# Arcadia-Science/arcadia-microscopy-tools

Hardware: AMD Instinct MI355X
Metric: fields-of-view/sec (4x2048^2 uint16) end-to-end segment+props (higher is better)
Workload: dtype f64; 1 GPU; configs[2]: synthetic 4-channel 2048x2048 uint16 FOVs, DAPI Gaussian+Otsu+open/close+EDT+peak markers+watershed nuclei (SEEDED relief, seeds_first: marker pixels spread first in raster order, cannot tie; SURVEY A.8's plain -EDT relief with exact ties is reported under sublines.a8_exact) + clear_border/relabel + morphology and 4-channel intensity regionprops; mode=weak scaling, 192 FOVs per GPU per step, streams_per_gpu=4, fovs_per_launch=48, max_cells_per_fov=2048, distinct_fovs_per_gpu=8, resident_in_hbm=True

## Files before the change

arcadia_microscopy_tools_amd/csrc/amt_common.h:

```cpp
#pragma once
#include <hip/hip_runtime.h>

#include <cstdarg>
#include <cstdint>
#include <cstdio>
#include <cstring>

#include "../../include/amt_hip.h"
#include "amt_scratch_plan.h"

struct amt_ctx {
    int device;
    hipStream_t stream;
    bool own_stream;
    char* arena;
    size_t arena_cap;
    char* mailbox;
    size_t mailbox_cap;
    size_t mailbox_off;
    int num_cus;
    hipStream_t aux[3];
    hipStream_t aux_own[3];
    hipEvent_t ev[4];
    bool aux_ready;
    int fork;
    size_t plan_off[AMT_SCRATCH_SLOTS];
    size_t plan_len[AMT_SCRATCH_SLOTS];
    int plan_count;
    size_t plan_total;
    bool plan_valid;
    unsigned long long* dbg_first;
};

int amt_fork(amt_ctx* ctx);
int amt_join(amt_ctx* ctx);

void amt_set_error(const char* fmt, ...);

#define AMT_HIP_CHECK(expr)                                                                      \
    do {                                                                                         \
        hipError_t _e = (expr);                                                                  \
        if (_e != hipSuccess) {                                                                  \
            amt_set_error("%s failed: %s (%s:%d)", #expr, hipGetErrorString(_e), __FILE__, __LINE__); \
            return AMT_EHIP;                                                                     \
        }                                                                                        \
    } while (0)

// ... 41 lines not shown
    for (long long v : f) {
        if (n > (SIZE_MAX >> 1) / (size_t)v) return SIZE_MAX >> 1;
        n *= (size_t)v;
    }
    return n;
}
static inline size_t amt_esize(int dtype) {
    switch (dtype) {
        case AMT_U8: return 1;
        case AMT_U16: return 2;
        case AMT_I32: case AMT_F32: return 4;
        case AMT_F64: case AMT_I64: return 8;
        default: return 0;
    }
}
int amt_check_operands(const char* op, const amt_operand* ops, int n);
#define AMT_CHECK_OPERANDS(op, ...)                                                              \
    do {                                                                                         \
        const amt_operand _ops[] = {__VA_ARGS__};                                                \
        AMT_TRY(amt_check_operands(op, _ops, (int)(sizeof(_ops) / sizeof(_ops[0]))));            \
    } while (0)

struct amt_scratch : amt_scratch_plan {
    amt_ctx* ctx;
    explicit amt_scratch(amt_ctx* c) : ctx(c) {}
    int commit();
};
int amt_param_upload(amt_ctx* ctx, void* dev_dst, const void* host_src, size_t bytes);

__host__ __device__ static inline size_t amt_align(size_t n, size_t a = 256) { return (n + a - 1) / a * a; }

static inline int amt_set_device(amt_ctx* ctx) {
    if (!ctx) {
        amt_set_error("null context");
        return AMT_EINVAL;
// ... 49 lines not shown
```

arcadia_microscopy_tools_amd/csrc/amt_ctx.hip:

```cpp
#include "amt_common.h"

#include <cstdlib>

static thread_local char g_err[1024] = "";

void amt_set_error(const char* fmt, ...) {
    va_list ap;
    va_start(ap, fmt);
    vsnprintf(g_err, sizeof(g_err), fmt, ap);
    va_end(ap);
}

int amt_check_operands(const char* op, const amt_operand* ops, int n) {
    for (int i = 0; i < n; ++i) {
        const amt_operand& a = ops[i];
        if (!a.ptr || !a.bytes) continue;
        const uintptr_t a0 = reinterpret_cast<uintptr_t>(a.ptr);
        const uintptr_t a1 = a.bytes > UINTPTR_MAX - a0 ? UINTPTR_MAX : a0 + a.bytes;
        for (int j = i + 1; j < n; ++j) {
            const amt_operand& b = ops[j];
            if (!b.ptr || !b.bytes || !(a.output || b.output)) continue;
            const uintptr_t b0 = reinterpret_cast<uintptr_t>(b.ptr);
            const uintptr_t b1 = b.bytes > UINTPTR_MAX - b0 ? UINTPTR_MAX : b0 + b.bytes;
            if (a1 <= b0 || b1 <= a0) continue;
            const amt_operand& o = a.output ? a : b;
            const amt_operand& x = a.output ? b : a;
            const bool allowed = (a.output && !b.output && ((a.inplace >> j) & 1u)) ||
                                 (b.output && !a.output && ((b.inplace >> i) & 1u));
// ... 67 lines not shown
    return AMT_OK;
}

extern "C" int amt_ctx_create(int device, amt_ctx** out) { return ctx_create_common(device, nullptr, true, out); }

extern "C" int amt_ctx_create_on_stream(int device, void* hip_stream, amt_ctx** out) {
    return ctx_create_common(device, (hipStream_t)hip_stream, false, out);
}

extern "C" int amt_ctx_destroy(amt_ctx* ctx) {
    if (!ctx) return AMT_OK;
    (void)hipSetDevice(ctx->device);
    (void)hipStreamSynchronize(ctx->stream);
    if (ctx->arena) (void)hipFree(ctx->arena);
    if (ctx->dbg_first) (void)hipFree(ctx->dbg_first);
    if (ctx->mailbox) (void)hipHostFree(ctx->mailbox);
    if (ctx->aux_ready) {
        for (int i = 0; i < 3; ++i) (void)hipStreamDestroy(ctx->aux_own[i]);
        for (int i = 0; i < 4; ++i) (void)hipEventDestroy(ctx->ev[i]);
    }
    if (ctx->own_stream) (void)hipStreamDestroy(ctx->stream);
    delete ctx;
    return AMT_OK;
}

extern "C" int amt_device_name(amt_ctx* ctx, char* buf, int buflen) {
    AMT_TRY(amt_set_device(ctx));
    AMT_REQUIRE(buf && buflen > 0, "amt_device_name: bad buffer");
    hipDeviceProp_t prop;
    AMT_HIP_CHECK(hipGetDeviceProperties(&prop, ctx->device));
    snprintf(buf, (size_t)buflen, "%s (%s, %d CUs)", prop.name, prop.gcnArchName, prop.multiProcessorCount);
    return AMT_OK;
}

static bool poison_enabled() {
    static int v = -1;
    if (v < 0) {
        const char* e = getenv("AMT_DEBUG_POISON");
        v = (e && e[0] == '1') ? 1 : 0;
    }
    return v == 1;
}

int amt_scratch::commit() {
    AMT_REQUIRE(!overflow, "scratch plan: more than %d buffers declared", AMT_SCRATCH_SLOTS);
    ctx->plan_valid = false;
    const size_t total_bytes = total + 4096;
    if (total_bytes > ctx->arena_cap) {
        AMT_HIP_CHECK(hipStreamSynchronize(ctx->stream));
        if (ctx->arena) AMT_HIP_CHECK(hipFree(ctx->arena));
        ctx->arena = nullptr;
        ctx->arena_cap = 0;
        size_t cap = total_bytes + total_bytes / 4;
        hipError_t e = hipMalloc((void**)&ctx->arena, cap);
        if (e != hipSuccess) {
            amt_set_error("scratch arena allocation of %zu bytes failed: %s", cap, hipGetErrorString(e));
// ... 116 lines not shown
        AMT_HIP_CHECK(hipStreamSynchronize(ctx->stream));
        return AMT_OK;
    }
    if (ctx->mailbox_off + need > ctx->mailbox_cap) {
        AMT_HIP_CHECK(hipStreamSynchronize(ctx->stream));
        ctx->mailbox_off = 0;
    }
    char* slot = ctx->mailbox + ctx->mailbox_off;
    ctx->mailbox_off += need;
    memcpy(slot, host_src, bytes);
    AMT_HIP_CHECK(hipMemcpyAsync(dev_dst, slot, bytes, hipMemcpyHostToDevice, ctx->stream));
    return AMT_OK;
}

extern "C" int amt_malloc(amt_ctx* ctx, size_t bytes, void** dptr) {
    AMT_TRY(amt_set_device(ctx));
    AMT_REQUIRE(dptr != nullptr, "amt_malloc: dptr is null");
    if (bytes == 0) bytes = 256;
    hipError_t e = hipMalloc(dptr, bytes);
    if (e != hipSuccess) {
        amt_set_error("hipMalloc(%zu) failed: %s", bytes, hipGetErrorString(e));
        return AMT_ENOMEM;
    }
    if (poison_enabled()) {
        AMT_HIP_CHECK(hipMemsetAsync(*dptr, 0xCD, bytes, ctx->stream));
        AMT_HIP_CHECK(hipStreamSynchronize(ctx->stream));
    }
    return AMT_OK;
}

extern "C" int amt_free(amt_ctx* ctx, void* dptr) {
    AMT_TRY(amt_set_device(ctx));
    if (dptr) AMT_HIP_CHECK(hipFree(dptr));
    return AMT_OK;
}

extern "C" int amt_memcpy_h2d(amt_ctx* ctx, void* dst, const void* src, size_t bytes) {
    AMT_TRY(amt_set_device(ctx));
    if (bytes) AMT_HIP_CHECK(hipMemcpyAsync(dst, src, bytes, hipMemcpyHostToDevice, ctx->stream));
    return AMT_OK;
}
extern "C" int amt_memcpy_d2h(amt_ctx* ctx, void* dst, const void* src, size_t bytes) {
    AMT_TRY(amt_set_device(ctx));
    if (bytes) AMT_HIP_CHECK(hipMemcpyAsync(dst, src, bytes, hipMemcpyDeviceToHost, ctx->stream));
    return AMT_OK;
}
extern "C" int amt_memcpy_d2d(amt_ctx* ctx, void* dst, const void* src, size_t bytes) {
    AMT_TRY(amt_set_device(ctx));
    if (bytes) AMT_HIP_CHECK(hipMemcpyAsync(dst, src, bytes, hipMemcpyDeviceToDevice, ctx->stream));
    return AMT_OK;
}
extern "C" int amt_memset(amt_ctx* ctx, void* dst, int value, size_t bytes) {
    AMT_TRY(amt_set_device(ctx));
    if (bytes) AMT_HIP_CHECK(hipMemsetAsync(dst, value, bytes, ctx->stream));
    return AMT_OK;
}
extern "C" int amt_sync(amt_ctx* ctx) {
    AMT_TRY(amt_set_device(ctx));
    AMT_HIP_CHECK(hipStreamSynchronize(ctx->stream));
    return AMT_OK;
}

extern "C" int amt_ctx_stream(amt_ctx* ctx, void** hip_stream) {
    AMT_REQUIRE(ctx && hip_stream, "amt_ctx_stream: null argument");
    *hip_stream = (void*)ctx->stream;
    return AMT_OK;
}

extern "C" int amt_stream_wait(amt_ctx* ctx, amt_ctx* other) {
    AMT_TRY(amt_set_device(ctx));
    AMT_REQUIRE(other != nullptr, "amt_stream_wait: other is null");
    AMT_REQUIRE(other->device == ctx->device, "amt_stream_wait: contexts on different devices");
    hipEvent_t ev;
    AMT_HIP_CHECK(hipEventCreateWithFlags(&ev, hipEventDisableTiming));
    AMT_HIP_CHECK(hipEventRecord(ev, other->stream));
    AMT_HIP_CHECK(hipStreamWaitEvent(ctx->stream, ev, 0));
    AMT_HIP_CHECK(hipEventDestroy(ev));
    return AMT_OK;
}

extern "C" int amt_event_create(amt_ctx* ctx, void** event) {
    AMT_TRY(amt_set_device(ctx));
    AMT_REQUIRE(event != nullptr, "amt_event_create: event is null");
    hipEvent_t ev;
    AMT_HIP_CHECK(hipEventCreateWithFlags(&ev, hipEventDisableTiming));
    *event = (void*)ev;
    return AMT_OK;
}
extern "C" int amt_event_record(amt_ctx* ctx, void* event) {
    AMT_TRY(amt_set_device(ctx));
    AMT_REQUIRE(event != nullptr, "amt_event_record: event is null");
    AMT_HIP_CHECK(hipEventRecord((hipEvent_t)event, ctx->stream));
    return AMT_OK;
}
extern "C" int amt_event_wait(amt_ctx* ctx, void* event) {
    AMT_TRY(amt_set_device(ctx));
    AMT_REQUIRE(event != nullptr, "amt_event_wait: event is null");
    AMT_HIP_CHECK(hipStreamWaitEvent(ctx->stream, (hipEvent_t)event, 0));
    return AMT_OK;
}
extern "C" int amt_event_sync(amt_ctx* ctx, void* event) {
    AMT_TRY(amt_set_device(ctx));
    AMT_REQUIRE(event != nullptr, "amt_event_sync: event is null");
    AMT_HIP_CHECK(hipEventSynchronize((hipEvent_t)event));
    return AMT_OK;
}
extern "C" int amt_event_destroy(amt_ctx* ctx, void* event) {
    AMT_TRY(amt_set_device(ctx));
    if (event) AMT_HIP_CHECK(hipEventDestroy((hipEvent_t)event));
    return AMT_OK;
}

extern "C" int amt_host_alloc(size_t bytes, void** hptr) {
    AMT_REQUIRE(hptr != nullptr, "amt_host_alloc: hptr is null");
    hipError_t e = hipHostMalloc(hptr, bytes ? bytes : 64, hipHostMallocDefault);
    if (e != hipSuccess) {
// ... 116 lines not shown
    AMT_HIP_CHECK(hipEventCreate(&t->stop));
    *timer = t;
    return AMT_OK;
}
extern "C" int amt_timer_start(amt_ctx* ctx, void* timer) {
    AMT_TRY(amt_set_device(ctx));
    AMT_HIP_CHECK(hipEventRecord(((amt_timer*)timer)->start, ctx->stream));
    return AMT_OK;
}
extern "C" int amt_timer_stop(amt_ctx* ctx, void* timer) {
    AMT_TRY(amt_set_device(ctx));
    AMT_HIP_CHECK(hipEventRecord(((amt_timer*)timer)->stop, ctx->stream));
    return AMT_OK;
}
extern "C" int amt_timer_elapsed_ms(amt_ctx* ctx, void* timer, float* ms) {
    AMT_TRY(amt_set_device(ctx));
    amt_timer* t = (amt_timer*)timer;
    AMT_HIP_CHECK(hipEventSynchronize(t->stop));
    AMT_HIP_CHECK(hipEventElapsedTime(ms, t->start, t->stop));
    return AMT_OK;
}
extern "C" int amt_timer_destroy(amt_ctx* ctx, void* timer) {
    AMT_TRY(amt_set_device(ctx));
    amt_timer* t = (amt_timer*)timer;
    if (t) {
        (void)hipEventDestroy(t->start);
        (void)hipEventDestroy(t->stop);
        delete t;
    }
    return AMT_OK;
// ... 2 lines not shown
```

arcadia_microscopy_tools_amd/csrc/amt_internal.h:

```cpp
#pragma once
#include "amt_common.h"

#include <type_traits>

template <int ITEMS>
__global__ void __launch_bounds__(1024) amt_scan_excl_kernel(int* __restrict__ data, int len, size_t plane_stride,
                                                             int* __restrict__ total,
                                                             const int* __restrict__ len_dev = nullptr) {
    __shared__ int s[1024];
    __shared__ int carry;
    int* d = data + (size_t)blockIdx.x * plane_stride;
    if (len_dev) len = len_dev[blockIdx.x];
    if (threadIdx.x == 0) carry = 0;
    __syncthreads();
    for (int start = 0; start < len; start += 1024 * ITEMS) {
        const int b = start + threadIdx.x * ITEMS;
        int v[ITEMS];
        int sum = 0;
#pragma unroll
        for (int k = 0; k < ITEMS; ++k) {
            v[k] = (b + k < len) ? d[b + k] : 0;
            sum += v[k];
        }
        s[threadIdx.x] = sum;
// ... 74 lines not shown
struct amt_runtabs {
    const unsigned long long* tbits;
    const unsigned short* roff;
    const unsigned short* rtab;
    const int* rcomp;
    int segs, trows;
};
int amt_i_propagate_roots(amt_ctx* ctx, const ccl_geom& g, int* A, const int* L, const int* rootlist, const int* nroots);

enum amt_comp_what { AMT_COMP_OBJECTS_BY_AREA, AMT_COMP_HOLES_BY_AREA, AMT_COMP_HOLES_BY_FRAME };
int amt_i_component_filter(amt_ctx* ctx, const uint8_t* in, uint8_t* out, int nplanes, int H, int W, bool c8,
                           amt_comp_what what, int size);

int amt_i_label_boxes(amt_ctx* ctx, const int* labels, int* bbox, unsigned long long* acc, int nplanes, int H, int W,
                      int max_label);
int amt_i_robust_intensity(amt_ctx* ctx, const int* labels, const int* bbox, const void* intensity, int in_code, int C,
                           double* wtable, int nplanes, int H, int W, int max_label);
int amt_i_relate_labels(amt_ctx* ctx, const int* labels, const int* bbox, const int* comp, int C, double* wtable,
                        int nplanes, int H, int W, int max_label);
int amt_i_neighbor_census(amt_ctx* ctx, const int* labels, const int* bbox, const int* comp, int C, double* wtable,
                          int nplanes, int H, int W, int max_label);
int amt_i_nearest_labels(amt_ctx* ctx, const double2* cen, double* wtable, int nplanes, int max_label);
int amt_i_texture(amt_ctx* ctx, const int32_t* labels, const void* intensity, int in_code, int C, const double* ranges,
                  int levels, int distance, bool counts, double* out, int nplanes, int H, int W, int max_label);
int amt_i_radial(amt_ctx* ctx, const int32_t* labels, const void* intensity, int in_code, int C, int bins, double* geom,
                 double* out, int nplanes, int H, int W, int max_label);

int amt_i_reconstruct(amt_ctx* ctx, const void* in, void* out, int dtype, int nplanes, int H, int W,
                      const uint8_t* footprint, int fh, int fw, int op, double cval, const void* minuend);

// ... 103 lines not shown
```

arcadia_microscopy_tools_amd/csrc/amt_overlay.hip:

```cpp
#include "amt_internal.h"

constexpr int OV_MAX_LAYERS = 8;

struct ov_params {
    const double* layer[OV_MAX_LAYERS];
    double opacity[OV_MAX_LAYERS];
    int mode[OV_MAX_LAYERS];
    int nlayers;
};

__device__ __forceinline__ double clip01(double v) { return v < 0.0 ? 0.0 : (v > 1.0 ? 1.0 : v); }

__global__ void __launch_bounds__(256) overlay_kernel(const double* __restrict__ bg, const ov_params* __restrict__ pp,
                                                      const double* __restrict__ luts, double* __restrict__ out,
                                                      size_t n) {
    extern __shared__ __attribute__((aligned(16))) char smem_raw[];
    double* lut = reinterpret_cast<double*>(smem_raw);
    __shared__ ov_params p;
    if (threadIdx.x == 0) p = *pp;
    __syncthreads();
    for (int i = threadIdx.x; i < p.nlayers * 1024; i += 256) lut[i] = luts[i];
    __syncthreads();
    for (size_t i = (size_t)blockIdx.x * 256 + threadIdx.x; i < n; i += (size_t)gridDim.x * 256) {
        const double b = clip01(bg[i]);
// ... 23 lines not shown
    }
}

extern "C" int amt_overlay(amt_ctx* ctx, const double* background, const double* const* layers_host, int nlayers,
                           const double* luts_host, const double* opacity_host, const int32_t* mode_host,
                           double* out_rgb, int H, int W) {
    {
        static const char* const lname[OV_MAX_LAYERS] = {"layers_host[0]", "layers_host[1]", "layers_host[2]", "layers_host[3]",
                                                         "layers_host[4]", "layers_host[5]", "layers_host[6]", "layers_host[7]"};
        amt_operand ops[2 + OV_MAX_LAYERS];
        int k = 0;
        ops[k++] = amt_in("background", background, amt_span(8, H, W));
        ops[k++] = amt_out("out_rgb", out_rgb, amt_span(8, H, W, 3));
        for (int l = 0; layers_host && l < nlayers && l < OV_MAX_LAYERS; ++l)
            ops[k++] = amt_in(lname[l], layers_host[l], amt_span(8, H, W));
        AMT_TRY(amt_check_operands("amt_overlay", ops, k));
    }
    AMT_TRY(amt_set_device(ctx));
    AMT_REQUIRE(background && out_rgb && H > 0 && W > 0, "overlay: bad arguments");
    AMT_REQUIRE(nlayers >= 0 && nlayers <= OV_MAX_LAYERS, "overlay: at most %d layers per call (got %d)", OV_MAX_LAYERS,
                nlayers);
    AMT_REQUIRE(nlayers == 0 || (layers_host && luts_host && opacity_host && mode_host), "overlay: null layer tables");
    ov_params hp;
    memset(&hp, 0, sizeof(hp));
    hp.nlayers = nlayers;
    for (int l = 0; l < nlayers; ++l) {
        AMT_REQUIRE(layers_host[l] != nullptr, "overlay: layer %d is null", l);
        AMT_REQUIRE(opacity_host[l] >= 0.0 && opacity_host[l] <= 1.0, "Opacity must be in [0, 1], got %g", opacity_host[l]);
        AMT_REQUIRE(mode_host[l] == 0 || mode_host[l] == 1, "overlay: blend mode must be 0 (alpha) or 1 (additive)");
        hp.layer[l] = layers_host[l];
        hp.opacity[l] = opacity_host[l];
// ... 16 lines not shown
```

arcadia_microscopy_tools_amd/csrc/amt_props.hip:

```cpp
#include "amt_internal.h"
#include "amt_perlabel.h"

#include <vector>

typedef unsigned long long u64;

enum { A_N = 0, A_SY, A_SX, A_SYY, A_SXX, A_SXY, A_C1, A_C2, A_C3, A_NACC };

__global__ void __launch_bounds__(256) rp_init_kernel(u64* __restrict__ acc, int* __restrict__ bbox, size_t nlab) {
    for (size_t i = (size_t)blockIdx.x * 256 + threadIdx.x; i < nlab; i += (size_t)gridDim.x * 256) {
        if (acc)
            for (int k = 0; k < A_NACC; ++k) acc[i * A_NACC + k] = 0;
        bbox[i * 4 + 0] = 0x7fffffff;
        bbox[i * 4 + 1] = 0x7fffffff;
        bbox[i * 4 + 2] = -1;
        bbox[i * 4 + 3] = -1;
    }
}

__device__ __forceinline__ double diff_of_products(u64 a, u64 b, u64 c, u64 d) {
    u64 lo1 = a * b, hi1 = __umul64hi(a, b);
    u64 lo2 = c * d, hi2 = __umul64hi(c, d);
    bool neg = (hi1 < hi2) || (hi1 == hi2 && lo1 < lo2);
    u64 hi, lo;
    if (!neg) {
        lo = lo1 - lo2;
        hi = hi1 - hi2 - (lo1 < lo2 ? 1 : 0);
    } else {
        lo = lo2 - lo1;
        hi = hi2 - hi1 - (lo2 < lo1 ? 1 : 0);
    }
    double v = (double)hi * 18446744073709551616.0 + (double)lo;
    return neg ? -v : v;
}

constexpr int BX_ROWS = 30, BX_COLS = 256, BX_BATCH = 4, BX_NBATCH = (BX_ROWS + 2) / BX_BATCH;
static_assert(BX_BATCH * BX_NBATCH == BX_ROWS + 2, "row batches must tile the strip");

template <bool VEC>
__global__ void __launch_bounds__(256) rp_boxes_kernel(const int* __restrict__ labels, int* __restrict__ bbox, int H,
                                                       int W, int max_label) {
    const int lane = threadIdx.x & 63;
    const int strip = blockIdx.x * 4 + (threadIdx.x >> 6);
    if (strip > (W - 1) / BX_COLS) return;
    const int plane = blockIdx.z;
    const int* L = labels + (size_t)plane * H * W;
    int* bbp = bbox + (size_t)plane * max_label * 4;
    const unsigned x = (unsigned)strip * BX_COLS + 4u * lane;
    const unsigned uw = (unsigned)W, ml = (unsigned)max_label;
    const int ya = blockIdx.y * BX_ROWS, yend = ya + BX_ROWS < H ? ya + BX_ROWS : H;

    unsigned xc[4], mlx[4];
#pragma unroll
    for (int k = 0; k < 4; ++k) {
        xc[k] = x + k < uw ? x + k : uw - 1u;
        mlx[k] = x + k < uw ? ml : 0u;
    }
    const unsigned xv = x < uw ? x : uw - 4u;
    auto load_row = [&](int y) -> int4 {
        const int yc = y < 0 ? 0 : (y < H ? y : H - 1);
// ... 50 lines not shown
                        if (q3[k]) atomicMax(&B[3], (int)(x + k));
                    }
                }
            }
#pragma unroll
            for (int k = 0; k < 6; ++k) {
                u[k] = c[k];
                c[k] = d[k];
            }
        }
#pragma unroll
        for (int j = 0; j < BX_BATCH; ++j) cur[j] = nxt[j];
    }
}

int amt_i_label_boxes(amt_ctx* ctx, const int* labels, int* bbox, unsigned long long* acc, int nplanes, int H, int W,
                      int max_label) {
    const size_t nlab = (size_t)nplanes * max_label;
    hipLaunchKernelGGL(rp_init_kernel, dim3(amt_grid_for(nlab, 256, 1024)), dim3(256), 0, ctx->stream, acc, bbox, nlab);
    AMT_LAUNCH_CHECK();
    const int nstrips = (W - 1) / BX_COLS + 1;
    const dim3 grid((nstrips + 3) / 4, (H - 1) / BX_ROWS + 1, nplanes);
    if ((uintptr_t)labels % 16 == 0 && W % 4 == 0)
        hipLaunchKernelGGL(rp_boxes_kernel<true>, grid, dim3(256), 0, ctx->stream, labels, bbox, H, W, max_label);
    else
        hipLaunchKernelGGL(rp_boxes_kernel<false>, grid, dim3(256), 0, ctx->stream, labels, bbox, H, W, max_label);
    AMT_LAUNCH_CHECK();
    return AMT_OK;
}

constexpr int RP_MAXC = 4;
constexpr int RPS = 3;
constexpr int RP_PW = 1024, RP_LBMAX = 7, RP_WIDE = 32 << RP_LBMAX;
__host__ __device__ constexpr int rp_band_rows(int lb) { return (RP_PW >> lb) - 4; }
__device__ __forceinline__ size_t rp_uniform(size_t v) {
    const unsigned lo = (unsigned)__builtin_amdgcn_readfirstlane((int)(unsigned)v);
    const unsigned hi = (unsigned)__builtin_amdgcn_readfirstlane((int)(unsigned)(v >> 32));
    return ((size_t)hi << 32) | lo;
}
struct RpSums {
    u64 cnt, sy, sx, syy, sxx, sxy;
    u64 s[RP_MAXC], q[RP_MAXC];
// ... 1483 lines not shown
```

arcadia_microscopy_tools_amd/csrc/amt_watershed.hip:

```cpp
#include "amt_internal.h"
#include <hip/hip_ext.h>

enum { CLS_NONE = 0, CLS_UNIFORM = 1, CLS_S = 3, CLS_M = 4, CLS_M2 = 5, CLS_L = 6, CLS_X = 7, CLS_G = 9 };
constexpr int WS_NLISTS = CLS_X - CLS_S + 1;
constexpr int WS_CTR = 24;
enum {
    WS_CTR_X = 0,
    WS_CTR_HBM = 7,
    WS_CTR_HASG = 8,
    WS_CTR_WL = 9,
    WS_CTR_NCOMP = 16
};
constexpr int S_PX = 2048, S_NB = 512;
constexpr int M_PX = 4096, M_NB = 512;
constexpr int M2_PX = 8192, M2_NB = 1024;
constexpr int L_PX = 24576, L_NB = 2048;
constexpr int X_PX = 32512, X_NB = 2048;

struct comp_row {
    int cmax;
    int mcnt;
    int x0, y0, x1, y1;
    int labmin, labmax;
    int cls;
    int root;
    int npix;
};

__global__ void __launch_bounds__(256) ws_seed_kernel(const int* __restrict__ markers, const int* __restrict__ L,
                                                      const int* __restrict__ F, int* __restrict__ out, size_t n,
                                                      const int* __restrict__ only_planes, amt_runtabs rt, int W) {
    if (only_planes && !only_planes[blockIdx.y]) return;
// ... 1544 lines not shown
                o.x = (unsigned)(vx - 1) < ml ? M[vx] : 0;
                o.y = (unsigned)(vy - 1) < ml ? M[vy] : 0;
                o.z = (unsigned)(vz - 1) < ml ? M[vz] : 0;
                o.w = (unsigned)(vw - 1) < ml ? M[vw] : 0;
            }
            *reinterpret_cast<int4*>(out + base + i0) = o;
        } else {
            for (size_t i = i0; i < n && i < i0 + 4; ++i) {
                const int v = ws_pixel_label(L[base + i], F, ws, base, i);
                out[base + i] = (unsigned)(v - 1) < ml ? M[v] : 0;
            }
        }
    }
}

__global__ void __launch_bounds__(1024) ws_label_map_kernel(const int* __restrict__ L, const int* __restrict__ F,
                                                            const int* __restrict__ ws, int* __restrict__ present,
                                                            const int* __restrict__ nlabels, int* __restrict__ count_dev,
                                                            int H, int W, int max_label, amt_runtabs rt) {
    __shared__ int s[1024];
    __shared__ int carry;
    const int plane = blockIdx.x;
    const size_t n = (size_t)H * W;
    const size_t base = (size_t)plane * n;
    int* P = present + (size_t)plane * (max_label + 1);
    const int k = nlabels[plane] < max_label ? nlabels[plane] : max_label;
    for (int l = threadIdx.x; l <= max_label; l += 1024) P[l] = (l >= 1 && l <= k) ? 1 : 0;
    __syncthreads();
    const int perim = 2 * W + 2 * H;
    for (int q = threadIdx.x; q < perim; q += 1024) {
        int y, x;
        if (q < W) {
            y = 0;
            x = q;
        } else if (q < 2 * W) {
            y = H - 1;
// ... 25 lines not shown
        __syncthreads();
        for (int off = 1; off < 1024; off <<= 1) {
            const int t = threadIdx.x >= off ? s[threadIdx.x - off] : 0;
            __syncthreads();
            s[threadIdx.x] += t;
            __syncthreads();
        }
        const int incl = s[threadIdx.x];
        const int c = carry;
        if (i <= max_label) P[i] = v ? c + incl : 0;
        __syncthreads();
        if (threadIdx.x == 1023) carry = c + incl;
        __syncthreads();
    }
    if (threadIdx.x == 0) count_dev[plane] = carry;
}

__global__ void __launch_bounds__(256) ws_final_map_kernel(int* __restrict__ Fall, const int* __restrict__ map,
                                                           const int* __restrict__ rootlist, const int* __restrict__ nroots,
                                                           size_t cap, size_t n, int max_label) {
    const int plane = blockIdx.z, shard = plane * gridDim.y + blockIdx.y;
    int* F = Fall + (size_t)plane * n;
    const int* M = map + (size_t)plane * (max_label + 1);
    const int cnt = nroots[shard] < (int)cap ? nroots[shard] : (int)cap;
    const int* lst = rootlist + (size_t)shard * cap;
    for (int k = blockIdx.x * 256 + threadIdx.x; k < cnt; k += gridDim.x * 256) {
        const int t = lst[k], f = F[t];
        F[t] = f > 0 ? ((unsigned)(f - 1) < (unsigned)max_label ? M[f] : 0) : (f == 0 ? -1 : 0);
    }
}
// ... 104 lines not shown
    const void* relief;
    bool use_d2;
    const int32_t* markers;
    const uint8_t* mask;
    int32_t* out;
    int nplanes, H, W, seeds_first;
    ws_fused fu;
    ccl_geom g;
    size_t n, row_stride, bstride;
    bool runs;
};
struct ws_bufs {
    int *L, *T, *moff, *boff, *cursor, *mlist, *next, *F, *rootlist, *nroots;
    comp_row* rows;
    int *btot, *mtot, *counters, *wl, *pf_idx, *pf_ctl, *ccl_scratch, *ties, *P;
    unsigned long long* tbits;
    unsigned short* rtab;
    int* nruns;
    unsigned short* roff;
    int *rcomp, *head, *tail;
    hp_elem *gheap, *heap;
    int *ncomp, *has_g, *wl_count;
    amt_runtabs rt;
};

static int ws_emulate(amt_ctx* ctx, const void* relief, bool use_d2, const int32_t* markers, const uint8_t* mask, int32_t* out,
                      hp_elem* gheap, const int* run, int nplanes, int H, int W, int conn) {
    const size_t n = (size_t)H * W;
    hipLaunchKernelGGL(ws_global_init_kernel, dim3(amt_grid_for(n, 256, 1024), nplanes), dim3(256), 0, ctx->stream, markers,
                       mask, out, run, n);
// ... 112 lines not shown
}

static int ws_flood_f64(const ws_args& a, const ws_bufs& b) {
    amt_ctx* ctx = a.ctx;
    hipLaunchKernelGGL(ws_flood_heap_kernel, dim3(64, a.nplanes), dim3(64), 0, ctx->stream, (const double*)a.relief, a.mask,
                       a.out, b.heap, b.mlist, b.rows, b.moff, b.boff, b.ncomp, b.counters + WS_CTR_HBM * a.nplanes,
                       a.row_stride, a.H, a.W, a.n, a.bstride, b.ties);
    AMT_LAUNCH_CHECK();
    return AMT_OK;
}

static int ws_fused_tail(const ws_args& a, const ws_bufs& b) {
    amt_ctx* ctx = a.ctx;
    const ccl_geom& g = a.g;
    const ws_fused& fu = a.fu;
    hipLaunchKernelGGL(ws_label_map_kernel, dim3(a.nplanes), dim3(1024), 0, ctx->stream, b.L, b.F, a.out, b.P, fu.nlabels_dev,
                       fu.count, a.H, a.W, fu.max_label, b.rt);
    AMT_LAUNCH_CHECK();
    if (a.runs) {
        hipLaunchKernelGGL(ws_final_map_kernel, g.glists, dim3(256), 0, ctx->stream, b.F, b.P, b.rootlist, b.nroots, g.cap, a.n,
                           fu.max_label);
        AMT_LAUNCH_CHECK();
        hipLaunchKernelGGL(ws_final_runs_kernel, dim3((unsigned)((g.ntiles + 3) / 4)), dim3(256), 0, ctx->stream, b.tbits, b.rtab,
                           b.nruns, b.F, a.out, b.P, fu.labels, a.H, a.W, g.segs, g.trows, (int)g.ntiles, fu.max_label);
    } else {
        hipLaunchKernelGGL(ws_final_kernel, dim3(amt_grid_for(a.n, 1024, 4096), a.nplanes), dim3(256), 0, ctx->stream, b.L, b.F,
                           a.out, b.P, fu.labels, a.n, fu.max_label);
    }
    AMT_LAUNCH_CHECK();
    return AMT_OK;
}

static int watershed_components(amt_ctx* ctx, const void* relief, bool use_d2, const int32_t* markers, const uint8_t* mask,
                                int32_t* out, int nplanes, int H, int W, int seeds_first, bool exact, int32_t* ties_dev,
                                const ws_fused& fu) {
    ws_args a = {ctx, relief, use_d2, markers, mask, out, nplanes, H, W, seeds_first, fu, amt_i_ccl_geom(nplanes, H, W)};
    const ccl_geom& g = a.g;
    const size_t n = a.n = g.n;
    const size_t np = (size_t)nplanes * n;
// ... 18 lines not shown
    amt_buf<comp_row> rows(s, nr);
    amt_buf<int> btot(s, nplanes);
    amt_buf<int> mtot(s, nplanes);
    amt_buf<int> counters(s, (size_t)nplanes * WS_CTR);
    amt_buf<int> wl(s, (size_t)WS_NLISTS * nr);
    amt_buf<int> pf_idx(s, (size_t)PF_NCLS * (nplanes + 1));
    amt_buf<int> pf_ctl(s, 16);
    amt_buf<int> ccl_scratch(s, g.multi_ints());
    amt_buf<int> ties_own(s, nplanes, !ties_dev);
    amt_buf<int> P(s, (size_t)nplanes * ((size_t)fu.max_label + 1), fu.labels != nullptr);
    amt_buf<unsigned long long> tbits(s, g.ntiles * 64, runs);
    amt_buf<unsigned short> rtab(s, g.ntiles * RT_CAP, runs);
    amt_buf<int> nruns(s, g.ntiles, runs);
    amt_buf<unsigned short> roff(s, g.ntiles * 64, runs);
    amt_buf<int> rcomp(s, g.ntiles * RT_CAP, runs);
    amt_buf<int> head(s, (size_t)nplanes * bstride, use_d2);
    amt_buf<int> tail(s, (size_t)nplanes * bstride, use_d2);
    amt_buf<hp_elem> gheap_own(s, np, use_d2 && exact);
    amt_buf<hp_elem> heap(s, (size_t)nplanes * bstride, !use_d2);
    AMT_TRY(s.commit());
    ws_bufs b = {};
    b.L = L, b.T = T, b.moff = moff, b.boff = boff, b.cursor = cursor, b.mlist = mlist, b.next = next, b.F = F;
    b.rootlist = rootlist, b.nroots = nroots, b.rows = rows, b.btot = btot, b.mtot = mtot, b.counters = counters, b.wl = wl;
    b.pf_idx = pf_idx, b.pf_ctl = pf_ctl, b.ccl_scratch = ccl_scratch, b.P = P;
    b.tbits = tbits, b.rtab = rtab, b.nruns = nruns, b.roff = roff, b.rcomp = rcomp, b.head = head, b.tail = tail;
    b.ties = ties_dev ? ties_dev : ties_own.p;
    b.heap = heap, b.gheap = use_d2 ? gheap_own.p : heap.p;
    b.ncomp = b.counters + WS_CTR_NCOMP * (size_t)nplanes;
    b.has_g = b.counters + WS_CTR_HASG * nplanes;
    b.wl_count = b.counters + WS_CTR_WL * nplanes;
    b.rt = {tbits, roff, rtab, rcomp, g.segs, g.trows};

    AMT_TRY(ws_label_and_classify(a, b));
    AMT_TRY(ws_prepare_hbm(a, b, fu.labels && use_d2));
    AMT_TRY(use_d2 ? ws_floods_d2(a, b) : ws_flood_f64(a, b));
    if (exact) AMT_TRY(ws_emulate(ctx, relief, use_d2, markers, mask, out, b.gheap, b.ties, nplanes, H, W, 1));
    if (fu.labels) AMT_TRY(ws_fused_tail(a, b));
    return AMT_OK;
}

// ... 70 lines not shown
```

Measured before the change: 16540 FOV/s.

## Compute label bounding boxes inside watershed tail and hand them to props

The fused watershed tail now computes per-label bounding boxes from component rows. Uniform components update their box directly, and flooded components are covered by a strip-walk kernel; planes that overflow fall back to a flagged full plane pass. The boxes are left in a context-owned buffer, and a serial-number handoff lets the next amt_i_label_boxes call copy them instead of rescanning every label plane. A poison/debug mode recomputes the boxes and compares them against the handed-over copy. This adds per-op bookkeeping and cross-call state that depends on the labels pointer and on the call order being exactly adjacent.

```diff
diff --git a/arcadia_microscopy_tools_amd/csrc/amt_common.h b/arcadia_microscopy_tools_amd/csrc/amt_common.h
--- a/arcadia_microscopy_tools_amd/csrc/amt_common.h
+++ b/arcadia_microscopy_tools_amd/csrc/amt_common.h
@@ -30,7 +30,23 @@
     size_t plan_total;
     bool plan_valid;
     unsigned long long* dbg_first;
+    unsigned long long op_serial;
+    int* box_buf;
+    size_t box_cap;
+    struct {
+        bool valid;
+        const void* labels;
+        int nplanes, H, W, max_label, device;
+        unsigned long long serial;
+    } box_note;
 };
+static inline void amt_note_op(amt_ctx* ctx) {
+    if (ctx) ++ctx->op_serial;
+}
+int amt_box_buffer(amt_ctx* ctx, size_t ints, int** buf);
+void amt_box_note_leave(amt_ctx* ctx, const void* labels, int nplanes, int H, int W, int max_label);
+const int* amt_box_note_take(amt_ctx* ctx, const void* labels, int nplanes, int H, int W, int max_label);
+bool amt_poison_enabled();
 
 int amt_fork(amt_ctx* ctx);
 int amt_join(amt_ctx* ctx);
@@ -102,11 +118,11 @@
         default: return 0;
     }
 }
-int amt_check_operands(const char* op, const amt_operand* ops, int n);
+int amt_check_operands(amt_ctx* ctx, const char* op, const amt_operand* ops, int n);
 #define AMT_CHECK_OPERANDS(op, ...)                                                              \
     do {                                                                                         \
         const amt_operand _ops[] = {__VA_ARGS__};                                                \
-        AMT_TRY(amt_check_operands(op, _ops, (int)(sizeof(_ops) / sizeof(_ops[0]))));            \
+        AMT_TRY(amt_check_operands(ctx, op, _ops, (int)(sizeof(_ops) / sizeof(_ops[0]))));       \
     } while (0)
 
 struct amt_scratch : amt_scratch_plan {
diff --git a/arcadia_microscopy_tools_amd/csrc/amt_ctx.hip b/arcadia_microscopy_tools_amd/csrc/amt_ctx.hip
--- a/arcadia_microscopy_tools_amd/csrc/amt_ctx.hip
+++ b/arcadia_microscopy_tools_amd/csrc/amt_ctx.hip
@@ -11,7 +11,8 @@
     va_end(ap);
 }
 
-int amt_check_operands(const char* op, const amt_operand* ops, int n) {
+int amt_check_operands(amt_ctx* ctx, const char* op, const amt_operand* ops, int n) {
+    amt_note_op(ctx);
     for (int i = 0; i < n; ++i) {
         const amt_operand& a = ops[i];
         if (!a.ptr || !a.bytes) continue;
@@ -109,6 +110,7 @@
     (void)hipStreamSynchronize(ctx->stream);
     if (ctx->arena) (void)hipFree(ctx->arena);
     if (ctx->dbg_first) (void)hipFree(ctx->dbg_first);
+    if (ctx->box_buf) (void)hipFree(ctx->box_buf);
     if (ctx->mailbox) (void)hipHostFree(ctx->mailbox);
     if (ctx->aux_ready) {
         for (int i = 0; i < 3; ++i) (void)hipStreamDestroy(ctx->aux_own[i]);
@@ -135,6 +137,39 @@
         v = (e && e[0] == '1') ? 1 : 0;
     }
     return v == 1;
+}
+bool amt_poison_enabled() { return poison_enabled(); }
+
+int amt_box_buffer(amt_ctx* ctx, size_t ints, int** buf) {
+    ctx->box_note.valid = false;
+    if (ints > ctx->box_cap) {
+        AMT_HIP_CHECK(hipStreamSynchronize(ctx->stream));
+        if (ctx->box_buf) AMT_HIP_CHECK(hipFree(ctx->box_buf));
+        ctx->box_buf = nullptr;
+        ctx->box_cap = 0;
+        const size_t cap = ints + ints / 4;
+        hipError_t e = hipMalloc((void**)&ctx->box_buf, cap * sizeof(int));
+        if (e != hipSuccess) {
+            amt_set_error("label box buffer allocation of %zu bytes failed: %s", cap * sizeof(int), hipGetErrorString(e));
+            return AMT_ENOMEM;
+        }
+        ctx->box_cap = cap;
+    }
+    *buf = ctx->box_buf;
+    return AMT_OK;
+}
+
+void amt_box_note_leave(amt_ctx* ctx, const void* labels, int nplanes, int H, int W, int max_label) {
+    if (!ctx->own_stream) return;
+    ctx->box_note = {true, labels, nplanes, H, W, max_label, ctx->device, ctx->op_serial};
+}
+
+const int* amt_box_note_take(amt_ctx* ctx, const void* labels, int nplanes, int H, int W, int max_label) {
+    const auto n = ctx->box_note;
+    ctx->box_note.valid = false;
+    const bool hit = n.valid && n.serial + 1 == ctx->op_serial && n.labels == labels && n.nplanes == nplanes && n.H == H &&
+                     n.W == W && n.max_label == max_label && n.device == ctx->device && ctx->box_buf;
+    return hit ? ctx->box_buf : nullptr;
 }
 
 int amt_scratch::commit() {
@@ -281,6 +316,7 @@
 }
 
 extern "C" int amt_malloc(amt_ctx* ctx, size_t bytes, void** dptr) {
+    amt_note_op(ctx);
     AMT_TRY(amt_set_device(ctx));
     AMT_REQUIRE(dptr != nullptr, "amt_malloc: dptr is null");
     if (bytes == 0) bytes = 256;
@@ -297,32 +333,38 @@
 }
 
 extern "C" int amt_free(amt_ctx* ctx, void* dptr) {
+    amt_note_op(ctx);
     AMT_TRY(amt_set_device(ctx));
     if (dptr) AMT_HIP_CHECK(hipFree(dptr));
     return AMT_OK;
 }
 
 extern "C" int amt_memcpy_h2d(amt_ctx* ctx, void* dst, const void* src, size_t bytes) {
+    amt_note_op(ctx);
     AMT_TRY(amt_set_device(ctx));
     if (bytes) AMT_HIP_CHECK(hipMemcpyAsync(dst, src, bytes, hipMemcpyHostToDevice, ctx->stream));
     return AMT_OK;
 }
 extern "C" int amt_memcpy_d2h(amt_ctx* ctx, void* dst, const void* src, size_t bytes) {
+    amt_note_op(ctx);
     AMT_TRY(amt_set_device(ctx));
     if (bytes) AMT_HIP_CHECK(hipMemcpyAsync(dst, src, bytes, hipMemcpyDeviceToHost, ctx->stream));
     return AMT_OK;
 }
 extern "C" int amt_memcpy_d2d(amt_ctx* ctx, void* dst, const void* src, size_t bytes) {
+    amt_note_op(ctx);
     AMT_TRY(amt_set_device(ctx));
     if (bytes) AMT_HIP_CHECK(hipMemcpyAsync(dst, src, bytes, hipMemcpyDeviceToDevice, ctx->stream));
     return AMT_OK;
 }
 extern "C" int amt_memset(amt_ctx* ctx, void* dst, int value, size_t bytes) {
+    amt_note_op(ctx);
     AMT_TRY(amt_set_device(ctx));
     if (bytes) AMT_HIP_CHECK(hipMemsetAsync(dst, value, bytes, ctx->stream));
     return AMT_OK;
 }
 extern "C" int amt_sync(amt_ctx* ctx) {
+    amt_note_op(ctx);
     AMT_TRY(amt_set_device(ctx));
     AMT_HIP_CHECK(hipStreamSynchronize(ctx->stream));
     return AMT_OK;
@@ -335,8 +377,10 @@
 }
 
 extern "C" int amt_stream_wait(amt_ctx* ctx, amt_ctx* other) {
+    amt_note_op(ctx);
     AMT_TRY(amt_set_device(ctx));
     AMT_REQUIRE(other != nullptr, "amt_stream_wait: other is null");
+    amt_note_op(other);
     AMT_REQUIRE(other->device == ctx->device, "amt_stream_wait: contexts on different devices");
     hipEvent_t ev;
     AMT_HIP_CHECK(hipEventCreateWithFlags(&ev, hipEventDisableTiming));
@@ -355,18 +399,21 @@
     return AMT_OK;
 }
 extern "C" int amt_event_record(amt_ctx* ctx, void* event) {
+    amt_note_op(ctx);
     AMT_TRY(amt_set_device(ctx));
     AMT_REQUIRE(event != nullptr, "amt_event_record: event is null");
     AMT_HIP_CHECK(hipEventRecord((hipEvent_t)event, ctx->stream));
     return AMT_OK;
 }
 extern "C" int amt_event_wait(amt_ctx* ctx, void* event) {
+    amt_note_op(ctx);
     AMT_TRY(amt_set_device(ctx));
     AMT_REQUIRE(event != nullptr, "amt_event_wait: event is null");
     AMT_HIP_CHECK(hipStreamWaitEvent(ctx->stream, (hipEvent_t)event, 0));
     return AMT_OK;
 }
 extern "C" int amt_event_sync(amt_ctx* ctx, void* event) {
+    amt_note_op(ctx);
     AMT_TRY(amt_set_device(ctx));
     AMT_REQUIRE(event != nullptr, "amt_event_sync: event is null");
     AMT_HIP_CHECK(hipEventSynchronize((hipEvent_t)event));
@@ -513,6 +560,7 @@
     return AMT_OK;
 }
 extern "C" int amt_timer_elapsed_ms(amt_ctx* ctx, void* timer, float* ms) {
+    amt_note_op(ctx);
     AMT_TRY(amt_set_device(ctx));
     amt_timer* t = (amt_timer*)timer;
     AMT_HIP_CHECK(hipEventSynchronize(t->stop));
diff --git a/arcadia_microscopy_tools_amd/csrc/amt_internal.h b/arcadia_microscopy_tools_amd/csrc/amt_internal.h
--- a/arcadia_microscopy_tools_amd/csrc/amt_internal.h
+++ b/arcadia_microscopy_tools_amd/csrc/amt_internal.h
@@ -112,6 +112,8 @@
 
 int amt_i_label_boxes(amt_ctx* ctx, const int* labels, int* bbox, unsigned long long* acc, int nplanes, int H, int W,
                       int max_label);
+int amt_i_label_boxes_flagged(amt_ctx* ctx, const int* labels, int* bbox, const int* only_planes, int nplanes, int H, int W,
+                              int max_label);
 int amt_i_robust_intensity(amt_ctx* ctx, const int* labels, const int* bbox, const void* intensity, int in_code, int C,
                            double* wtable, int nplanes, int H, int W, int max_label);
 int amt_i_relate_labels(amt_ctx* ctx, const int* labels, const int* bbox, const int* comp, int C, double* wtable,
diff --git a/arcadia_microscopy_tools_amd/csrc/amt_overlay.hip b/arcadia_microscopy_tools_amd/csrc/amt_overlay.hip
--- a/arcadia_microscopy_tools_amd/csrc/amt_overlay.hip
+++ b/arcadia_microscopy_tools_amd/csrc/amt_overlay.hip
@@ -61,7 +61,7 @@
         ops[k++] = amt_out("out_rgb", out_rgb, amt_span(8, H, W, 3));
         for (int l = 0; layers_host && l < nlayers && l < OV_MAX_LAYERS; ++l)
             ops[k++] = amt_in(lname[l], layers_host[l], amt_span(8, H, W));
-        AMT_TRY(amt_check_operands("amt_overlay", ops, k));
+        AMT_TRY(amt_check_operands(ctx, "amt_overlay", ops, k));
     }
     AMT_TRY(amt_set_device(ctx));
     AMT_REQUIRE(background && out_rgb && H > 0 && W > 0, "overlay: bad arguments");
diff --git a/arcadia_microscopy_tools_amd/csrc/amt_props.hip b/arcadia_microscopy_tools_amd/csrc/amt_props.hip
--- a/arcadia_microscopy_tools_amd/csrc/amt_props.hip
+++ b/arcadia_microscopy_tools_amd/csrc/amt_props.hip
@@ -7,15 +7,22 @@
 
 enum { A_N = 0, A_SY, A_SX, A_SYY, A_SXX, A_SXY, A_C1, A_C2, A_C3, A_NACC };
 
-__global__ void __launch_bounds__(256) rp_init_kernel(u64* __restrict__ acc, int* __restrict__ bbox, size_t nlab) {
+__global__ void __launch_bounds__(256) rp_init_kernel(u64* __restrict__ acc, int* __restrict__ bbox, size_t nlab,
+                                                      const int* __restrict__ src) {
     for (size_t i = (size_t)blockIdx.x * 256 + threadIdx.x; i < nlab; i += (size_t)gridDim.x * 256) {
         if (acc)
             for (int k = 0; k < A_NACC; ++k) acc[i * A_NACC + k] = 0;
-        bbox[i * 4 + 0] = 0x7fffffff;
-        bbox[i * 4 + 1] = 0x7fffffff;
-        bbox[i * 4 + 2] = -1;
-        bbox[i * 4 + 3] = -1;
-    }
+        bbox[i * 4 + 0] = src ? src[i * 4 + 0] : 0x7fffffff;
+        bbox[i * 4 + 1] = src ? src[i * 4 + 1] : 0x7fffffff;
+        bbox[i * 4 + 2] = src ? src[i * 4 + 2] : -1;
+        bbox[i * 4 + 3] = src ? src[i * 4 + 3] : -1;
+    }
+}
+
+__global__ void __launch_bounds__(256) rp_boxes_differ_kernel(const int* __restrict__ a, const int* __restrict__ b, size_t n,
+                                                              u64* __restrict__ first) {
+    for (size_t i = (size_t)blockIdx.x * 256 + threadIdx.x; i < n; i += (size_t)gridDim.x * 256)
+        if (a[i] != b[i]) atomicMin(first, (u64)i);
 }
 
 __device__ __forceinline__ double diff_of_products(u64 a, u64 b, u64 c, u64 d) {
@@ -39,11 +46,12 @@
 
 template <bool VEC>
 __global__ void __launch_bounds__(256) rp_boxes_kernel(const int* __restrict__ labels, int* __restrict__ bbox, int H,
-                                                       int W, int max_label) {
+                                                       int W, int max_label, const int* __restrict__ only_planes) {
     const int lane = threadIdx.x & 63;
     const int strip = blockIdx.x * 4 + (threadIdx.x >> 6);
     if (strip > (W - 1) / BX_COLS) return;
     const int plane = blockIdx.z;
+    if (only_planes && !only_planes[plane]) return;
     const int* L = labels + (size_t)plane * H * W;
     int* bbp = bbox + (size_t)plane * max_label * 4;
     const unsigned x = (unsigned)strip * BX_COLS + 4u * lane;
@@ -124,18 +132,49 @@
     }
 }
 
+static int rp_boxes_pass(amt_ctx* ctx, const int* labels, int* bbox, int nplanes, int H, int W, int max_label,
+                         const int* only_planes) {
+    const int nstrips = (W - 1) / BX_COLS + 1;
+    const dim3 grid((nstrips + 3) / 4, (H - 1) / BX_ROWS + 1, nplanes);
+    if ((uintptr_t)labels % 16 == 0 && W % 4 == 0)
+        hipLaunchKernelGGL(rp_boxes_kernel<true>, grid, dim3(256), 0, ctx->stream, labels, bbox, H, W, max_label, only_planes);
+    else
+        hipLaunchKernelGGL(rp_boxes_kernel<false>, grid, dim3(256), 0, ctx->stream, labels, bbox, H, W, max_label, only_planes);
+    AMT_LAUNCH_CHECK();
+    return AMT_OK;
+}
+
+int amt_i_label_boxes_flagged(amt_ctx* ctx, const int* labels, int* bbox, const int* only_planes, int nplanes, int H, int W,
+                              int max_label) {
+    return rp_boxes_pass(ctx, labels, bbox, nplanes, H, W, max_label, only_planes);
+}
+
 int amt_i_label_boxes(amt_ctx* ctx, const int* labels, int* bbox, unsigned long long* acc, int nplanes, int H, int W,
                       int max_label) {
     const size_t nlab = (size_t)nplanes * max_label;
-    hipLaunchKernelGGL(rp_init_kernel, dim3(amt_grid_for(nlab, 256, 1024)), dim3(256), 0, ctx->stream, acc, bbox, nlab);
+    const int* handed = amt_box_note_take(ctx, labels, nplanes, H, W, max_label);
+    const bool check = handed && amt_poison_enabled();
+    hipLaunchKernelGGL(rp_init_kernel, dim3(amt_grid_for(nlab, 256, 1024)), dim3(256), 0, ctx->stream, acc, bbox, nlab,
+                       check ? (const int*)nullptr : handed);
     AMT_LAUNCH_CHECK();
-    const int nstrips = (W - 1) / BX_COLS + 1;
-    const dim3 grid((nstrips + 3) / 4, (H - 1) / BX_ROWS + 1, nplanes);
-    if ((uintptr_t)labels % 16 == 0 && W % 4 == 0)
-        hipLaunchKernelGGL(rp_boxes_kernel<true>, grid, dim3(256), 0, ctx->stream, labels, bbox, H, W, max_label);
-    else
-        hipLaunchKernelGGL(rp_boxes_kernel<false>, grid, dim3(256), 0, ctx->stream, labels, bbox, H, W, max_label);
-    AMT_LAUNCH_CHECK();
+    if (handed && !check) return AMT_OK;
+    AMT_TRY(rp_boxes_pass(ctx, labels, bbox, nplanes, H, W, max_label, nullptr));
+    if (check) {
+        if (!ctx->dbg_first) AMT_HIP_CHECK(hipMalloc((void**)&ctx->dbg_first, sizeof(unsigned long long)));
+        AMT_HIP_CHECK(hipMemsetAsync(ctx->dbg_first, 0xFF, sizeof(unsigned long long), ctx->stream));
+        hipLaunchKernelGGL(rp_boxes_differ_kernel, dim3(amt_grid_for(nlab * 4, 256, 1024)), dim3(256), 0, ctx->stream, handed,
+                           (const int*)bbox, nlab * 4, ctx->dbg_first);
+        AMT_LAUNCH_CHECK();
+        unsigned long long first = 0;
+        AMT_HIP_CHECK(hipMemcpyAsync(&first, ctx->dbg_first, sizeof(first), hipMemcpyDeviceToHost, ctx->stream));
+        AMT_HIP_CHECK(hipStreamSynchronize(ctx->stream));
+        if (first != ~0ull) {
+            amt_set_error("label boxes: the boxes handed over by amt_watershed_edt_cleared differ from the plane pass at "
+                          "plane %llu, label %llu, field %llu",
+                          first / 4 / (unsigned long long)max_label, first / 4 % (unsigned long long)max_label + 1, first % 4);
+            return AMT_EHIP;
+        }
+    }
     return AMT_OK;
 }
 
diff --git a/arcadia_microscopy_tools_amd/csrc/amt_watershed.hip b/arcadia_microscopy_tools_amd/csrc/amt_watershed.hip
--- a/arcadia_microscopy_tools_amd/csrc/amt_watershed.hip
+++ b/arcadia_microscopy_tools_amd/csrc/amt_watershed.hip
@@ -16,6 +16,7 @@
 constexpr int M2_PX = 8192, M2_NB = 1024;
 constexpr int L_PX = 24576, L_NB = 2048;
 constexpr int X_PX = 32512, X_NB = 2048;
+constexpr int WS_BOX_BLOCKS = 64, WS_BOX_ROWS = 32;
 
 struct comp_row {
     int cmax;
@@ -1590,12 +1591,23 @@
     }
 }
 
+struct ws_box_args {
+    int* bbox;
+    const comp_row* rows;
+    const int* ncomp;
+    size_t row_stride;
+    int2* flist;
+    int* fcount;
+    int* fbig;
+};
+
 __global__ void __launch_bounds__(1024) ws_label_map_kernel(const int* __restrict__ L, const int* __restrict__ F,
                                                             const int* __restrict__ ws, int* __restrict__ present,
                                                             const int* __restrict__ nlabels, int* __restrict__ count_dev,
-                                                            int H, int W, int max_label, amt_runtabs rt) {
+                                                            int H, int W, int max_label, amt_runtabs rt, ws_box_args bx) {
     __shared__ int s[1024];
     __shared__ int carry;
+    __shared__ int nwalk, big;
     const int plane = blockIdx.x;
     const size_t n = (size_t)H * W;
     const size_t base = (size_t)plane * n;
@@ -1651,6 +1663,91 @@
         __syncthreads();
     }
     if (threadIdx.x == 0) count_dev[plane] = carry;
+    if (!bx.bbox) return;
+    int* B = bx.bbox + (size_t)plane * max_label * 4;
+    for (int i = threadIdx.x; i < max_label * 4; i += 1024) B[i] = (i & 2) ? -1 : 0x7fffffff;
+    if (threadIdx.x == 0) nwalk = 0, big = 0;
+    __syncthreads();
+    const comp_row* rows = bx.rows + (size_t)plane * bx.row_stride;
+    const int fcap = (int)(bx.row_stride / 2);
+    int2* fl = bx.flist + (size_t)plane * fcap;
+    const int nc = bx.ncomp[plane];
+    for (int i = threadIdx.x; i < nc; i += 1024) {
+        const comp_row c = rows[i];
+        if (c.cls == CLS_UNIFORM) {
+            const int m = (unsigned)(c.labmin - 1) < (unsigned)max_label ? P[c.labmin] : 0;
+            if (m > 0) {
+                int* b = B + (size_t)(m - 1) * 4;
+                atomicMin(&b[0], c.y0);
+                atomicMin(&b[1], c.x0);
+                atomicMax(&b[2], c.y1);
+                atomicMax(&b[3], c.x1);
+            }
+        } else if (c.cls >= CLS_S) {
+            const long long area = (long long)(c.x1 - c.x0 + 3) * (c.y1 - c.y0 + 3);
+            const int nb = (c.y1 - c.y0) / WS_BOX_ROWS + 1, nch = (c.x1 - c.x0) / 64 + 1;
+            const int at = area > X_PX ? fcap : atomicAdd(&nwalk, nb * nch);
+            if (area > X_PX || at > fcap - nb * nch) {
+                big = 1;
+            } else {
+                for (int k = 0; k < nb * nch; ++k) fl[at + k] = make_int2(i, (k % nb) | ((k / nb) << 16));
+            }
+        }
+    }
+    __syncthreads();
+    if (threadIdx.x == 0) bx.fcount[plane] = big ? 0 : nwalk, bx.fbig[plane] = big;
+}
+
+__global__ void __launch_bounds__(256) ws_flood_boxes_kernel(const int* __restrict__ labels, ws_box_args bx, int H, int W,
+                                                             int max_label) {
+    const int lane = threadIdx.x & 63;
+    const int plane = blockIdx.y;
+    const int cnt = bx.fcount[plane];
+    const int* Lp = labels + (size_t)plane * H * W;
+    int* B = bx.bbox + (size_t)plane * max_label * 4;
+    const comp_row* rows = bx.rows + (size_t)plane * bx.row_stride;
+    const int2* fl = bx.flist + (size_t)plane * (bx.row_stride / 2);
+    const unsigned ml = (unsigned)max_label;
+    constexpr int FQ = 4;
+    for (int j = blockIdx.x * 4 + (threadIdx.x >> 6); j < cnt; j += gridDim.x * 4) {
+        const int2 it = fl[j];
+        const comp_row c = rows[it.x];
+        const int ya = c.y0 + (it.y & 0xffff) * WS_BOX_ROWS;
+        const int yb = ya + WS_BOX_ROWS - 1 < c.y1 ? ya + WS_BOX_ROWS - 1 : c.y1;
+        const int x = c.x0 + (it.y >> 16) * 64 + lane;
+        const bool in = x <= c.x1;
+        const int xl = in ? x : c.x1;
+        auto load = [&](int y) -> int {
+            int v = 0;
+            if (in && y >= 0 && y < H && y <= yb + 1) v = Lp[(size_t)y * W + xl];
+            return (unsigned)(v - 1) < ml ? v : 0;
+        };
+        int up = load(ya - 1), cur = load(ya);
+        for (int y = ya; y <= yb; y += FQ) {
+            int nx[FQ];
+#pragma unroll
+            for (int q = 0; q < FQ; ++q) nx[q] = load(y + 1 + q);
+#pragma unroll
+            for (int q = 0; q < FQ; ++q) {
+                const int yy = y + q;
+                if (yy > yb) break;
+                const int dn = nx[q];
+                const int l = amt_lane_left(cur), r = amt_lane_right(cur);
+                const int ul = amt_lane_left(up), ur = amt_lane_right(up);
+                const int dl = amt_lane_left(dn), dr = amt_lane_right(dn);
+                if (cur) {
+                    int* b = B + (size_t)(cur - 1) * 4;
+                    const bool head = l != cur, tail = r != cur;
+                    if (head && up != cur) atomicMin(&b[0], yy);
+                    if (head && dn != cur) atomicMax(&b[2], yy);
+                    if (head && ul != cur && dl != cur) atomicMin(&b[1], x);
+                    if (tail && ur != cur && dr != cur) atomicMax(&b[3], x);
+                }
+                up = cur;
+                cur = dn;
+            }
+        }
+    }
 }
 
 __global__ void __launch_bounds__(256) ws_final_map_kernel(int* __restrict__ Fall, const int* __restrict__ map,
@@ -1785,6 +1882,7 @@
     int *L, *T, *moff, *boff, *cursor, *mlist, *next, *F, *rootlist, *nroots;
     comp_row* rows;
     int *btot, *mtot, *counters, *wl, *pf_idx, *pf_ctl, *ccl_scratch, *ties, *P;
+    int* fctl;
     unsigned long long* tbits;
     unsigned short* rtab;
     int* nruns;
@@ -1927,8 +2025,14 @@
     amt_ctx* ctx = a.ctx;
     const ccl_geom& g = a.g;
     const ws_fused& fu = a.fu;
+    ws_box_args bx = {};
+    if (a.runs && fu.max_label > 0 && ctx->own_stream) {
+        AMT_TRY(amt_box_buffer(ctx, (size_t)a.nplanes * fu.max_label * 4, &bx.bbox));
+        bx.rows = b.rows, bx.ncomp = b.ncomp, bx.row_stride = a.row_stride;
+        bx.flist = reinterpret_cast<int2*>(b.cursor), bx.fcount = b.fctl, bx.fbig = b.fctl + a.nplanes;
+    }
     hipLaunchKernelGGL(ws_label_map_kernel, dim3(a.nplanes), dim3(1024), 0, ctx->stream, b.L, b.F, a.out, b.P, fu.nlabels_dev,
-                       fu.count, a.H, a.W, fu.max_label, b.rt);
+                       fu.count, a.H, a.W, fu.max_label, b.rt, bx);
     AMT_LAUNCH_CHECK();
     if (a.runs) {
         hipLaunchKernelGGL(ws_final_map_kernel, g.glists, dim3(256), 0, ctx->stream, b.F, b.P, b.rootlist, b.nroots, g.cap, a.n,
@@ -1936,6 +2040,14 @@
         AMT_LAUNCH_CHECK();
         hipLaunchKernelGGL(ws_final_runs_kernel, dim3((unsigned)((g.ntiles + 3) / 4)), dim3(256), 0, ctx->stream, b.tbits, b.rtab,
                            b.nruns, b.F, a.out, b.P, fu.labels, a.H, a.W, g.segs, g.trows, (int)g.ntiles, fu.max_label);
+        if (bx.bbox) {
+            AMT_LAUNCH_CHECK();
+            hipLaunchKernelGGL(ws_flood_boxes_kernel, dim3(WS_BOX_BLOCKS, a.nplanes), dim3(256), 0, ctx->stream,
+                               (const int*)fu.labels, bx, a.H, a.W, fu.max_label);
+            AMT_LAUNCH_CHECK();
+            AMT_TRY(amt_i_label_boxes_flagged(ctx, fu.labels, bx.bbox, bx.fbig, a.nplanes, a.H, a.W, fu.max_label));
+            amt_box_note_leave(ctx, fu.labels, a.nplanes, a.H, a.W, fu.max_label);
+        }
     } else {
         hipLaunchKernelGGL(ws_final_kernel, dim3(amt_grid_for(a.n, 1024, 4096), a.nplanes), dim3(256), 0, ctx->stream, b.L, b.F,
                            a.out, b.P, fu.labels, a.n, fu.max_label);
@@ -1984,6 +2096,7 @@
     amt_buf<int> nruns(s, g.ntiles, runs);
     amt_buf<unsigned short> roff(s, g.ntiles * 64, runs);
     amt_buf<int> rcomp(s, g.ntiles * RT_CAP, runs);
+    amt_buf<int> fctl(s, (size_t)2 * nplanes, runs);
     amt_buf<int> head(s, (size_t)nplanes * bstride, use_d2);
     amt_buf<int> tail(s, (size_t)nplanes * bstride, use_d2);
     amt_buf<hp_elem> gheap_own(s, np, use_d2 && exact);
@@ -1994,6 +2107,7 @@
     b.rootlist = rootlist, b.nroots = nroots, b.rows = rows, b.btot = btot, b.mtot = mtot, b.counters = counters, b.wl = wl;
     b.pf_idx = pf_idx, b.pf_ctl = pf_ctl, b.ccl_scratch = ccl_scratch, b.P = P;
     b.tbits = tbits, b.rtab = rtab, b.nruns = nruns, b.roff = roff, b.rcomp = rcomp, b.head = head, b.tail = tail;
+    b.fctl = fctl;
     b.ties = ties_dev ? ties_dev : ties_own.p;
     b.heap = heap, b.gheap = use_d2 ? gheap_own.p : heap.p;
     b.ncomp = b.counters + WS_CTR_NCOMP * (size_t)nplanes;
```

Result: faster. 17220 FOV/s (median of 6 runs) (+4.1%).
